# UT-Austin-RPL/GIGA

Hardware: AMD Instinct MI355X
Metric: scenes/sec (higher is better)
Workload: dtype f32; 1 GPU; c2: batch=32/GPU synthetic 40^3 TSDF, encoder + 3 grasp heads @1 query + occupancy head @2048 queries/scene (literal train_giga call), fp32 MFMA; parallelism=scene-sharded x1 (scene i -> rank i mod 1; replicas, no data-path collective)

## Files before the change

### giga_amd/csrc/giga_wino.h

```cpp
#pragma once
#include "giga_conv16.h"

namespace giga {

constexpr unsigned WINO_DEFAULT_MASK = 0xFFF;
constexpr int WINO_NW = 8;
constexpr int WINO_PS = 80;
template <int H, int W> struct WinoBlock {
    static constexpr int TW = W / 2, TH = H / 2;
    static constexpr int BW = TW % 4 == 0 ? 4 : 5, BH = TW % 4 == 0 ? 4 : 3;
    static constexpr int TXB = (TW + BW - 1) / BW, TYB = (TH + BH - 1) / BH;
    static constexpr int PW = 2 * BW + 2, PH = 2 * BH + 2;
    static constexpr int RS = BW == 4 ? 832 : 1040;
    static constexpr int REGION = PH * RS;
    static_assert(BW * BH <= 16 && PW * WINO_PS <= RS, "tile block");
};
constexpr int wino_kpass(int cin) { return cin > 64 ? cin / 64 : 1; }
template <int C0, int C1, int H, int W>
constexpr int wino_nw() {
    constexpr int CINP = (C0 + C1) / wino_kpass(C0 + C1);
    constexpr int fit = (160 * 1024 - 16 * CINP * 16 * 4) / WinoBlock<H, W>::REGION;
    return fit >= WINO_NW ? WINO_NW : (fit / 2) * 2;
}
template <int C0, int C1, int H, int W>
constexpr size_t wino_lds_bytes() {
    constexpr int CINP = (C0 + C1) / wino_kpass(C0 + C1);
    return (size_t)16 * CINP * 16 * 4 + (size_t)wino_nw<C0, C1, H, W>() * WinoBlock<H, W>::REGION;
}
constexpr size_t wino_image_bytes(int cin, int cout) { return (size_t)16 * cin * cout * 4; }

__device__ __forceinline__ void store_f32x4(float* uniform_base, unsigned byte_off, f32x4v v) {
    *reinterpret_cast<f32x4v*>(reinterpret_cast<char*>(uniform_base) + byte_off) = v;
}

template <int C0, int C1, int COUT>
__device__ __forceinline__ void wino_fill(const ConvArgs& a, uint8_t* smem, int block, int nblocks, int kpass) {
    constexpr int CIN = C0 + C1, KP = wino_kpass(CIN), CINP = CIN / KP, NGRP = COUT / 16;
    constexpr int WFRAGS = 16 * (CINP / 16);
    const int lane = threadIdx.x & 63;
    const int wave = __builtin_amdgcn_readfirstlane(threadIdx.x >> 6);
    const int nwl = blockDim.x >> 6;
    const int grp = conv_wg_map<NGRP>(a, block, nblocks).grp;
    const uint8_t* wsrc = a.w + ((size_t)grp * KP + kpass) * WFRAGS * FRAG;
    for (int c = wave; c < WFRAGS; c += nwl)
        __builtin_amdgcn_global_load_lds(
            (const __attribute__((address_space(1))) void*)(wsrc + (size_t)c * FRAG + lane * 16),
            (__attribute__((address_space(3))) void*)(smem + c * FRAG), 16, 0, 0);
}

template <int C0, int C1, int COUT, int H, int W, bool POOL, bool RELU>
__device__ __forceinline__ void wino_run(const ConvArgs& a, uint8_t* smem, int block, int nblocks, int kpass) {
    using G = WinoBlock<H, W>;
    constexpr int CIN = C0 + C1, KP = wino_kpass(CIN), CINP = CIN / KP, NCHUNK = CINP / 16, NGRP = COUT / 16;
    constexpr int NWV = wino_nw<C0, C1, H, W>();
    constexpr int BW = G::BW, BH = G::BH, PW = G::PW, PH = G::PH, RS = G::RS, PS = WINO_PS, REGION = G::REGION;
    constexpr int NVEC = PW * PH * 4, NLD = (NVEC + 63) / 64;
    constexpr int WBYTES = 16 * CINP * 16 * 4;
    static_assert(C1 == 0 || (C0 % 16 == 0 && (KP == 1 || C0 % CINP == 0)), "concat boundary on a chunk / pass boundary");
    static_assert(!POOL || KP == 1, "pooled layers are single-pass");
    static_assert(KP <= 2, "a third pass would read partials back through an L1 line it has read before");

    const int lane = threadIdx.x & 63;
    const int wave = __builtin_amdgcn_readfirstlane(threadIdx.x >> 6);
    const int j = lane & 15, g = lane >> 4;
    const bool active = wave < NWV;
    CONV_T(0);
    uint8_t* region = smem + WBYTES + (active ? wave : 0) * REGION;
    const ConvWgMap wm = conv_wg_map<NGRP>(a, block, nblocks);
    const int grp = wm.grp, wg_in_grp = wm.wg_in_grp, wgs_per_grp = wm.wgs_per_grp;
    const int units_all = wm.nimg * G::TYB * G::TXB;
    const int ulo = (int)((long long)units_all * wg_in_grp / wgs_per_grp), uhi = (int)((long long)units_all * (wg_in_grp + 1) / wgs_per_grp);
    const int units = uhi;
    const bool klast = kpass == KP - 1;

    const int jt = j < BW * BH ? j : 0;
    const int tyl = jt / BW, txl = jt % BW;
    const int a_off = 2 * tyl * RS + 2 * txl * PS + 16 * g;

    const int v16 = (lane & 3) * 16;
    const uint32_t rowb = (uint32_t)(a.cs0 ? a.cs0 : C0) * 4;
    constexpr uint32_t OOB = 0x80000000u;
    int st_lds[NLD];
    uint32_t st_rel[NLD];
#pragma unroll
    for (int q = 0; q < NLD; ++q) {
        const int i = lane + 64 * q, pix = i >> 2, ly = pix / PW, lx = pix % PW;
        st_lds[q] = i < NVEC ? ly * RS + lx * PS + v16 : 64;
        st_rel[q] = i < NVEC ? (uint32_t)(ly * W + lx) * rowb + (uint32_t)v16 : OOB;
    }
    const uint32_t in_bytes = (uint32_t)a.nimg * H * W * rowb;
    const __amdgpu_buffer_rsrc_t rs0 = __builtin_amdgcn_make_buffer_rsrc(
        const_cast<char*>(reinterpret_cast<const char*>(a.in0)) + (size_t)a.co0 * 4, 0, in_bytes, 0x00020000);
    const __amdgpu_buffer_rsrc_t rs1 = C1 > 0 ? __builtin_amdgcn_make_buffer_rsrc(
        const_cast<char*>(reinterpret_cast<const char*>(a.in1)) + (size_t)a.co1 * 4, 0, in_bytes, 0x00020000) : rs0;
    auto unit_coords = [&](int u, int& bx, int& by, int& img) {
        bx = u % G::TXB; by = (u / G::TXB) % G::TYB; img = wm.img0 + u / (G::TXB * G::TYB);
    };
    typedef unsigned u32x4v __attribute__((ext_vector_type(4)));
    u32x4v stg[NLD];
    uint32_t st_off[NLD];
    auto unit_setup = [&](int u) {
        int bx, by, img;
        unit_coords(u, bx, by, img);
        const int y0 = 2 * BH * by - 1, x0 = 2 * BW * bx - 1;
        const uint32_t base = (uint32_t)((img * H + y0) * W + x0) * rowb;
        if (y0 >= 0 && x0 >= 0 && y0 + PH <= H && x0 + PW <= W) {
#pragma unroll
            for (int q = 0; q < NLD; ++q) st_off[q] = (64 * (q + 1) > NVEC && st_rel[q] == OOB) ? OOB : st_rel[q] + base;
        } else {
#pragma unroll
            for (int q = 0; q < NLD; ++q) {
                const int pix = (lane >> 2) + 16 * q;
                const int ly = (pix * (65536 / PW + 1)) >> 16, lx = pix - ly * PW;
                const bool ok = st_rel[q] != OOB && (unsigned)(y0 + ly) < (unsigned)H && (unsigned)(x0 + lx) < (unsigned)W;
                st_off[q] = ok ? st_rel[q] + base : OOB;
            }
        }
    };
    auto issue_loads = [&](int cc) {
        const int c16 = kpass * CINP + cc * 16;
        const bool first = C1 == 0 || c16 < C0;
        const int soff = (first ? c16 : c16 - C0) * 4;
#pragma unroll
        for (int q = 0; q < NLD; ++q)
            stg[q] = first ? __builtin_amdgcn_raw_buffer_load_b128(rs0, st_off[q], soff, 0)
                           : __builtin_amdgcn_raw_buffer_load_b128(rs1, st_off[q], soff, 0);
    };

    int u = ulo + wave;
    const bool work = active && u < units;
    if (work) { unit_setup(u); issue_loads(0); }
    const f32x4v bias4 = (a.bias && klast) ? *reinterpret_cast<const f32x4v*>(a.bias + grp * 16 + 4 * g) : f32x4v{0.f, 0.f, 0.f, 0.f};
    __builtin_amdgcn_s_waitcnt(0x0F70);
    __syncthreads();
    if (!work) return;
    CONV_T(1);
    int tcount = 2;

    f32x4v acc[16];
    const uint8_t* wl = smem + lane * 8;
    float* outp = reinterpret_cast<float*>(a.out);

    auto epilogue = [&](const int u) {
        int bx, by, img;
        unit_coords(u, bx, by, img);
        const int ty = BH * by + tyl, tx = BW * bx + txl;
        const bool ok = j < BW * BH && ty < G::TH && tx < G::TW;
        f32x4v t0[4], t1[4];
#pragma unroll
        for (int xi = 0; xi < 4; ++xi) {
            t0[xi] = (acc[4 * xi] + acc[4 * xi + 1]) + acc[4 * xi + 2];
            t1[xi] = acc[4 * xi + 1] - (acc[4 * xi + 2] + acc[4 * xi + 3]);
        }
        f32x4v y[4];
        y[0] = (t0[0] + t0[1]) + t0[2]; y[1] = (t1[0] + t1[1]) + t1[2];
        y[2] = t0[1] - (t0[2] + t0[3]); y[3] = t1[1] - (t1[2] + t1[3]);
        const uint32_t pix = (uint32_t)((img * H + 2 * ty) * W + 2 * tx);
        const uint32_t o00 = (pix * COUT + grp * 16 + 4 * g) * 4u;
        if (ok) {
#pragma unroll
            for (int e = 0; e < 4; ++e) {
                const uint32_t off = o00 + (uint32_t)(((e >> 1) * W + (e & 1)) * COUT * 4);
                if constexpr (KP > 1) {
                    if (kpass > 0) y[e] += *reinterpret_cast<const f32x4v*>(reinterpret_cast<const char*>(outp) + off);
                }
                if (klast) {
                    if (RELU) {
#pragma unroll
                        for (int r = 0; r < 4; ++r) y[e][r] = relu(y[e][r]);
                    } else if (a.mask) {
                        const f32x4v mk = *reinterpret_cast<const f32x4v*>(reinterpret_cast<const char*>(a.mask) + off);
#pragma unroll
                        for (int r = 0; r < 4; ++r) y[e][r] = mk[r] > 0.f ? y[e][r] : 0.f;
                    }
                }
                store_f32x4(outp, off, y[e]);
            }
            if constexpr (POOL) {
                f32x4v mx;
#pragma unroll
                for (int r = 0; r < 4; ++r) mx[r] = fmaxf(fmaxf(y[0][r], y[1][r]), fmaxf(y[2][r], y[3][r]));
                const uint32_t pp = (uint32_t)((img * (H / 2) + ty) * (W / 2) + tx);
                store_f32x4(reinterpret_cast<float*>(a.out_pool), (pp * COUT + grp * 16 + 4 * g) * 4u, mx);
            }
        }
    };

    f32x2v d[4][4];
    auto load_d = [&](const int h) {
#pragma unroll
        for (int r = 0; r < 4; ++r)
#pragma unroll
            for (int x = 0; x < 4; ++x)
                d[r][x] = *(const volatile __attribute__((address_space(3))) f32x2v*)(region + a_off + r * RS + x * PS + 8 * h);
    };
    auto stage_write = [&]() {
#pragma unroll
        for (int q = 0; q < NLD; ++q) *reinterpret_cast<u32x4v*>(region + st_lds[q]) = stg[q];
    };
    f32x2v v[16];
    auto transform = [&]() {
#pragma unroll
        for (int x = 0; x < 4; ++x) {
            const f32x2v e0 = d[0][x] - d[2][x], e1 = d[1][x] + d[2][x], e2 = d[2][x] - d[1][x], e3 = d[1][x] - d[3][x];
            d[0][x] = e0; d[1][x] = e1; d[2][x] = e2; d[3][x] = e3;
        }
#pragma unroll
        for (int xi = 0; xi < 4; ++xi) {
            v[4 * xi + 0] = d[xi][0] - d[xi][2];
            v[4 * xi + 1] = d[xi][1] + d[xi][2];
            v[4 * xi + 2] = d[xi][2] - d[xi][1];
            v[4 * xi + 3] = d[xi][1] - d[xi][3];
        }
    };
    auto burst = [&](auto first_tag, const int cc, const int h, auto&& mid) {
        constexpr bool FIRST = decltype(first_tag)::value;
        const uint8_t* wbase = wl + (cc * 2 + h) * 512;
        constexpr int PD = 4;
        f32x2v wq[PD][2];
#pragma unroll
        for (int pp = 0; pp < PD; ++pp) {
            wq[pp][0] = *reinterpret_cast<const f32x2v*>(wbase + (2 * pp) * NCHUNK * 1024);
            wq[pp][1] = *reinterpret_cast<const f32x2v*>(wbase + (2 * pp + 1) * NCHUNK * 1024);
        }
        __builtin_amdgcn_sched_barrier(0);
#pragma unroll
        for (int pp = 0; pp < 8; ++pp) {
            const int sl = pp % PD, p0 = 2 * pp, p1 = 2 * pp + 1;
            if constexpr (FIRST) {
                acc[p0] = mfma32_16(wq[sl][0][0], v[p0][0], f32x4v{0.f, 0.f, 0.f, 0.f});
                acc[p1] = mfma32_16(wq[sl][1][0], v[p1][0], p1 == 5 ? bias4 : f32x4v{0.f, 0.f, 0.f, 0.f});
            } else {
                acc[p0] = mfma32_16(wq[sl][0][0], v[p0][0], acc[p0]);
                acc[p1] = mfma32_16(wq[sl][1][0], v[p1][0], acc[p1]);
            }
            acc[p0] = mfma32_16(wq[sl][0][1], v[p0][1], acc[p0]);
            acc[p1] = mfma32_16(wq[sl][1][1], v[p1][1], acc[p1]);
            __builtin_amdgcn_sched_barrier(0);
            if (pp + PD < 8) {
                wq[sl][0] = *reinterpret_cast<const f32x2v*>(wbase + (2 * (pp + PD)) * NCHUNK * 1024);
                wq[sl][1] = *reinterpret_cast<const f32x2v*>(wbase + (2 * (pp + PD) + 1) * NCHUNK * 1024);
            }
            if (pp == 3) mid();
            __builtin_amdgcn_sched_barrier(0);
        }
    };

    static_assert(NCHUNK >= 2, "loads run two chunks ahead");
    stage_write();
    issue_loads(1);
    load_d(0);
    while (true) {
        const int un = u + NWV;
        const bool more = un < units;
#pragma unroll
        for (int cc = 0; cc < NCHUNK; ++cc) {
            transform();
            auto mid0 = [&]() { load_d(1); };
            if (cc == 0) burst(std::true_type{}, cc, 0, mid0); else burst(std::false_type{}, cc, 0, mid0);
            if (cc == 0) { CONV_T(tcount); ++tcount; }
            transform();
            auto mid1 = [&]() {
                if (cc + 1 < NCHUNK) {
                    stage_write();
                    if (cc + 2 < NCHUNK) issue_loads(cc + 2);
                    else if (more) { unit_setup(un); issue_loads(0); }
                    load_d(0);
                } else if (more) {
                    stage_write();
                    issue_loads(1);
                    load_d(0);
                }
            };
            burst(std::false_type{}, cc, 1, mid1);
        }
        epilogue(u);
        CONV_T(tcount); ++tcount;
        if (!more) break;
        u = un;
    }
    CONV_T(63);
}

template <int C0, int C1, int COUT, int H, int W, bool POOL, bool RELU>
__global__ __launch_bounds__((wino_nw<C0, C1, H, W>() * 64)) void wino_kernel(ConvArgs a) {
    extern __shared__ __attribute__((aligned(16))) uint8_t smem[];
    constexpr int KP = wino_kpass(C0 + C1);
#pragma unroll
    for (int k = 0; k < KP; ++k) {
        if (k > 0) {
            __builtin_amdgcn_s_waitcnt(0x0F70);
            __syncthreads();
        }
        wino_fill<C0, C1, COUT>(a, smem, (int)blockIdx.x, (int)gridDim.x, k);
        wino_run<C0, C1, COUT, H, W, POOL, RELU>(a, smem, (int)blockIdx.x, (int)gridDim.x, k);
    }
}

template <int CIN, int COUT>
__device__ __forceinline__ void up_fill(const ConvArgs& a, uint8_t* smem, int block, int nblocks) {
    constexpr int KG = CIN / 16, NBT = COUT / 16;
    const int lane = threadIdx.x & 63;
    const int wave = __builtin_amdgcn_readfirstlane(threadIdx.x >> 6);
    const int nwl = blockDim.x >> 6;
    const int grp = conv_wg_map<NBT>(a, block, nblocks).grp;
    for (int c = wave; c < 4 * KG; c += nwl) {
        const int sub = c / KG, kg = c - sub * KG;
        __builtin_amdgcn_global_load_lds(
            (const __attribute__((address_space(1))) void*)(a.w + ((size_t)(sub * NBT + grp) * KG + kg) * FRAG + lane * 16),
            (__attribute__((address_space(3))) void*)(smem + c * FRAG), 16, 0, 0);
    }
}
template <int CIN, int COUT, int H, int W>
__device__ __forceinline__ void up_run(const ConvArgs& a, uint8_t* smem, int block, int nblocks) {
    constexpr int KG = CIN / 16, NBT = COUT / 16, NWV = WINO_NW;
    const int lane = threadIdx.x & 63;
    const int wave = __builtin_amdgcn_readfirstlane(threadIdx.x >> 6);
    const int j = lane & 15, g = lane >> 4;
    const bool active = wave < NWV;
    const ConvWgMap wm = conv_wg_map<NBT>(a, block, nblocks);
    const int grp = wm.grp;
    const int npix = wm.nimg * H * W, p0 = wm.img0 * H * W;
    const int units_all = (npix + 15) / 16;
    const int ulo = (int)((long long)units_all * wm.wg_in_grp / wm.wgs_per_grp), uhi = (int)((long long)units_all * (wm.wg_in_grp + 1) / wm.wgs_per_grp);
    const uint32_t rowb = (uint32_t)(a.cs0 ? a.cs0 : CIN) * 4;
    const char* in = reinterpret_cast<const char*>(a.in0) + (size_t)a.co0 * 4 + 16 * g;
    f32x4v x[2][KG];
    auto issue = [&](int u, f32x4v (&dst)[KG]) {
        int p = 16 * u + j;
        p = p < npix ? p : npix - 1;
        const char* q = in + (size_t)(p0 + p) * rowb;
#pragma unroll
        for (int k = 0; k < KG; ++k) dst[k] = *reinterpret_cast<const f32x4v*>(q + 64 * k);
    };
    int u = ulo + wave;
    const bool work = active && u < uhi;
    if (work) issue(u, x[0]);
    const f32x4v bias4 = a.bias ? *reinterpret_cast<const f32x4v*>(a.bias + grp * 16 + 4 * g) : f32x4v{0.f, 0.f, 0.f, 0.f};
    __builtin_amdgcn_s_waitcnt(0x0F70);
    __syncthreads();
    if (!work) return;
    const f32x4v* wl = reinterpret_cast<const f32x4v*>(smem) + lane;
    float* outp = reinterpret_cast<float*>(a.out);
    auto unit = [&](const int u, const f32x4v (&xb)[KG]) {
        f32x4v acc[4];
#pragma unroll
        for (int k = 0; k < KG; ++k) {
            f32x4v wv[4];
#pragma unroll
            for (int sub = 0; sub < 4; ++sub) wv[sub] = wl[(sub * KG + k) * 64];
#pragma unroll
            for (int e = 0; e < 4; ++e)
#pragma unroll
                for (int sub = 0; sub < 4; ++sub)
                    acc[sub] = (k == 0 && e == 0) ? mfma32_16(wv[sub][e], xb[k][e], bias4) : mfma32_16(wv[sub][e], xb[k][e], acc[sub]);
        }
        const int p = 16 * u + j;
        if (p < npix) {
            const int pg = p0 + p, img = pg / (H * W), r = pg - img * (H * W), y = r / W, xx = r - y * W;
            const uint32_t o00 = ((uint32_t)((img * 2 * H + 2 * y) * 2 * W + 2 * xx) * COUT + grp * 16 + 4 * g) * 4u;
#pragma unroll
            for (int sub = 0; sub < 4; ++sub)
                store_f32x4(outp, o00 + (uint32_t)(((sub >> 1) * 2 * W + (sub & 1)) * COUT * 4), acc[sub]);
        }
    };
    while (true) {
        const int un = u + NWV;
        const bool more = un < uhi;
        if (more) issue(un, x[1]);
        unit(u, x[0]);
        if (!more) break;
        const int un2 = un + NWV;
        const bool more2 = un2 < uhi;
        if (more2) issue(un2, x[0]);
        unit(un, x[1]);
        if (!more2) break;
        u = un2;
    }
}
template <int CIN, int COUT>
constexpr size_t up_lds_bytes() { return (size_t)4 * (CIN / 16) * FRAG; }
template <int CIN, int COUT, int H, int W>
__global__ __launch_bounds__(WINO_NW * 64) void up_kernel(ConvArgs a) {
    extern __shared__ __attribute__((aligned(16))) uint8_t smem[];
    up_fill<CIN, COUT>(a, smem, (int)blockIdx.x, (int)gridDim.x);
    up_run<CIN, COUT, H, W>(a, smem, (int)blockIdx.x, (int)gridDim.x);
}
template <int CIN, int COUT, int H, int W>
inline int launch_up(const ConvArgs& a, hipStream_t s) {
    constexpr int NBT = COUT / 16;
    constexpr size_t lds = up_lds_bytes<CIN, COUT>();
    const size_t in_pix = (size_t)a.nimg * H * W;
    if (in_pix * 4 >= (1u << 24) || in_pix * 4 * COUT * 4 >= (1ull << 32)) return -7;
    const int units = (int)((in_pix + 15) / 16);
    int wgs = (units + WINO_NW - 1) / WINO_NW;
    if (wgs > 256 / NBT) wgs = 256 / NBT;
    else if (a.xcd_local && a.nimg % 8 == 0 && wgs % 8 != 0 && wgs + 8 - wgs % 8 <= 256 / NBT) wgs += 8 - wgs % 8;
    auto kern = up_kernel<CIN, COUT, H, W>;
    if (lds > 48 * 1024) giga::dyn_lds_once(reinterpret_cast<const void*>(kern), (int)lds);
    GIGA_LAUNCH(kern, dim3(wgs * NBT), dim3(WINO_NW * 64), lds, s, a);
    return hipGetLastError() == hipSuccess ? 0 : -10;
}

template <int C0, int C1, int COUT, int H, int W, bool POOL, bool RELU = true>
inline int launch_wino(const ConvArgs& a, hipStream_t s) {
    using G = WinoBlock<H, W>;
    constexpr int NWV = wino_nw<C0, C1, H, W>(), NGRP = COUT / 16;
    constexpr size_t lds = wino_lds_bytes<C0, C1, H, W>();
    static_assert(lds <= 160 * 1024 && NWV >= 4, "LDS budget");
    static_assert(256 % NGRP == 0, "weight groups must divide the CU count");
    const size_t in_pix = (size_t)a.nimg * H * W;
    if (C1 > 0 && (a.cs0 ? a.cs0 : C0) != (a.cs1 ? a.cs1 : C1)) return -7;
    if (in_pix * (size_t)((a.cs0 ? a.cs0 : C0) * 4) >= (1ull << 31)) return -7;
    if (in_pix >= (1u << 24) || in_pix * (size_t)((a.cs0 ? a.cs0 : C0) * 4) >= (1ull << 32) ||
        (C1 > 0 && in_pix * (size_t)((a.cs1 ? a.cs1 : C1) * 4) >= (1ull << 32)) || in_pix * COUT * 4 >= (1ull << 32)) return -7;
    const int units = a.nimg * G::TXB * G::TYB;
    int wgs = (units + NWV - 1) / NWV;
    if (wgs > 256 / NGRP) wgs = 256 / NGRP;
    else if (a.xcd_local && a.nimg % 8 == 0 && wgs % 8 != 0 && wgs + 8 - wgs % 8 <= 256 / NGRP) wgs += 8 - wgs % 8;
    auto kern = wino_kernel<C0, C1, COUT, H, W, POOL, RELU>;
    if (lds > 48 * 1024) giga::dyn_lds_once(reinterpret_cast<const void*>(kern), (int)lds);
    GIGA_LAUNCH(kern, dim3(wgs * NGRP), dim3(NWV * 64), lds, s, a);
    return hipGetLastError() == hipSuccess ? 0 : -10;
}

}
```

Before: 98200 scenes/s.

## Precompute per-boundary-class halo load offsets in an LDS table for Winograd conv

Per-unit computation of halo-load offsets and bounds checks is replaced by a small LDS table, one entry per boundary class (first, interior, last block in x and y). Each unit now adds a per-unit scalar base and reads its offsets from the table ahead of time. The buffer resource base is shifted back by one row plus one pixel so the offsets stay non-negative. The output transform is split into paired 2-wide ops with asm barriers to steer codegen, and the `more` test is recomputed through an opaque asm. The table costs extra LDS, which may lower the wave count in LDS-bound configurations.

```diff
diff --git a/giga_amd/csrc/giga_wino.h b/giga_amd/csrc/giga_wino.h
--- a/giga_amd/csrc/giga_wino.h
+++ b/giga_amd/csrc/giga_wino.h
@@ -14,21 +14,29 @@
     static constexpr int RS = BW == 4 ? 832 : 1040;
     static constexpr int REGION = PH * RS;
     static_assert(BW * BH <= 16 && PW * WINO_PS <= RS, "tile block");
+    static constexpr int NCX = TXB < 3 ? TXB : 3, NCY = TYB < 3 ? TYB : 3, NCLS = NCX * NCY;
+    static constexpr int NLD = (PW * PH * 4 + 63) / 64;
+    static constexpr int TAB = NCLS * NLD * 256;
+    static constexpr int cls(int b, int nb, int nc) { return b == 0 ? 0 : b == nb - 1 ? nc - 1 : 1; }
+    static constexpr int rep(int c, int nb, int nc) { return c == 0 ? 0 : c == nc - 1 ? nb - 1 : 1; }
+    static_assert((TXB < 3 || (2 * BW - 1 >= 0 && 2 * BW * (TXB - 2) - 1 + PW <= W)) &&
+                  (TYB < 3 || (2 * BH - 1 >= 0 && 2 * BH * (TYB - 2) - 1 + PH <= H)), "blocks between the first and the last lie inside the image");
 };
 constexpr int wino_kpass(int cin) { return cin > 64 ? cin / 64 : 1; }
 template <int C0, int C1, int H, int W>
 constexpr int wino_nw() {
     constexpr int CINP = (C0 + C1) / wino_kpass(C0 + C1);
-    constexpr int fit = (160 * 1024 - 16 * CINP * 16 * 4) / WinoBlock<H, W>::REGION;
+    constexpr int fit = (160 * 1024 - 16 * CINP * 16 * 4 - WinoBlock<H, W>::TAB) / WinoBlock<H, W>::REGION;
     return fit >= WINO_NW ? WINO_NW : (fit / 2) * 2;
 }
 template <int C0, int C1, int H, int W>
 constexpr size_t wino_lds_bytes() {
     constexpr int CINP = (C0 + C1) / wino_kpass(C0 + C1);
-    return (size_t)16 * CINP * 16 * 4 + (size_t)wino_nw<C0, C1, H, W>() * WinoBlock<H, W>::REGION;
+    return (size_t)16 * CINP * 16 * 4 + (size_t)wino_nw<C0, C1, H, W>() * WinoBlock<H, W>::REGION + WinoBlock<H, W>::TAB;
 }
 constexpr size_t wino_image_bytes(int cin, int cout) { return (size_t)16 * cin * cout * 4; }
 
+__device__ __forceinline__ f32x2v pair_of(f32x4v a, int hh) { return hh ? f32x2v{a[2], a[3]} : f32x2v{a[0], a[1]}; }
 __device__ __forceinline__ void store_f32x4(float* uniform_base, unsigned byte_off, f32x4v v) {
     *reinterpret_cast<f32x4v*>(reinterpret_cast<char*>(uniform_base) + byte_off) = v;
 }
@@ -54,7 +62,7 @@
     constexpr int CIN = C0 + C1, KP = wino_kpass(CIN), CINP = CIN / KP, NCHUNK = CINP / 16, NGRP = COUT / 16;
     constexpr int NWV = wino_nw<C0, C1, H, W>();
     constexpr int BW = G::BW, BH = G::BH, PW = G::PW, PH = G::PH, RS = G::RS, PS = WINO_PS, REGION = G::REGION;
-    constexpr int NVEC = PW * PH * 4, NLD = (NVEC + 63) / 64;
+    constexpr int NVEC = PW * PH * 4, NLD = G::NLD;
     constexpr int WBYTES = 16 * CINP * 16 * 4;
     static_assert(C1 == 0 || (C0 % 16 == 0 && (KP == 1 || C0 % CINP == 0)), "concat boundary on a chunk / pass boundary");
     static_assert(!POOL || KP == 1, "pooled layers are single-pass");
@@ -81,55 +89,83 @@
     const uint32_t rowb = (uint32_t)(a.cs0 ? a.cs0 : C0) * 4;
     constexpr uint32_t OOB = 0x80000000u;
     int st_lds[NLD];
-    uint32_t st_rel[NLD];
 #pragma unroll
     for (int q = 0; q < NLD; ++q) {
         const int i = lane + 64 * q, pix = i >> 2, ly = pix / PW, lx = pix % PW;
         st_lds[q] = i < NVEC ? ly * RS + lx * PS + v16 : 64;
-        st_rel[q] = i < NVEC ? (uint32_t)(ly * W + lx) * rowb + (uint32_t)v16 : OOB;
-    }
-    const uint32_t in_bytes = (uint32_t)a.nimg * H * W * rowb;
+    }
+    auto st_entry = [&](int q, int x0, int y0) -> uint32_t {
+        const int i = lane + 64 * q, pix = i >> 2;
+        const int ly = (pix * (65536 / PW + 1)) >> 16, lx = pix - ly * PW;
+        const bool ok = i < NVEC && (unsigned)(y0 + ly) < (unsigned)H && (unsigned)(x0 + lx) < (unsigned)W;
+        return ok ? (uint32_t)(ly * W + lx) * rowb + (uint32_t)v16 : OOB;
+    };
+    const uint32_t front = (uint32_t)(W + 1) * rowb;
+    const uint32_t in_bytes = (uint32_t)a.nimg * H * W * rowb + front;
     const __amdgpu_buffer_rsrc_t rs0 = __builtin_amdgcn_make_buffer_rsrc(
-        const_cast<char*>(reinterpret_cast<const char*>(a.in0)) + (size_t)a.co0 * 4, 0, in_bytes, 0x00020000);
+        const_cast<char*>(reinterpret_cast<const char*>(a.in0)) + (size_t)a.co0 * 4 - front, 0, in_bytes, 0x00020000);
     const __amdgpu_buffer_rsrc_t rs1 = C1 > 0 ? __builtin_amdgcn_make_buffer_rsrc(
-        const_cast<char*>(reinterpret_cast<const char*>(a.in1)) + (size_t)a.co1 * 4, 0, in_bytes, 0x00020000) : rs0;
+        const_cast<char*>(reinterpret_cast<const char*>(a.in1)) + (size_t)a.co1 * 4 - front, 0, in_bytes, 0x00020000) : rs0;
     auto unit_coords = [&](int u, int& bx, int& by, int& img) {
         bx = u % G::TXB; by = (u / G::TXB) % G::TYB; img = wm.img0 + u / (G::TXB * G::TYB);
+    };
+    auto unit_base = [&](int u) -> uint32_t {
+        int bx, by, img;
+        unit_coords(u, bx, by, img);
+        return (uint32_t)((img * H + 2 * BH * by) * W + 2 * BW * bx) * rowb;
+    };
+    constexpr int TAB0 = WBYTES + NWV * REGION;
+    typedef const __attribute__((address_space(3))) uint32_t* tab_ptr;
+    const tab_ptr tab_lane = (tab_ptr)(smem + TAB0 + lane * 4);
+    auto unit_tab = [&](int u) -> tab_ptr {
+        int bx, by, img;
+        unit_coords(u, bx, by, img);
+        return tab_lane + (G::cls(by, G::TYB, G::NCY) * G::NCX + G::cls(bx, G::TXB, G::NCX)) * (NLD * 64);
     };
     typedef unsigned u32x4v __attribute__((ext_vector_type(4)));
     u32x4v stg[NLD];
     uint32_t st_off[NLD];
-    auto unit_setup = [&](int u) {
-        int bx, by, img;
-        unit_coords(u, bx, by, img);
-        const int y0 = 2 * BH * by - 1, x0 = 2 * BW * bx - 1;
-        const uint32_t base = (uint32_t)((img * H + y0) * W + x0) * rowb;
-        if (y0 >= 0 && x0 >= 0 && y0 + PH <= H && x0 + PW <= W) {
-#pragma unroll
-            for (int q = 0; q < NLD; ++q) st_off[q] = (64 * (q + 1) > NVEC && st_rel[q] == OOB) ? OOB : st_rel[q] + base;
-        } else {
-#pragma unroll
-            for (int q = 0; q < NLD; ++q) {
-                const int pix = (lane >> 2) + 16 * q;
-                const int ly = (pix * (65536 / PW + 1)) >> 16, lx = pix - ly * PW;
-                const bool ok = st_rel[q] != OOB && (unsigned)(y0 + ly) < (unsigned)H && (unsigned)(x0 + lx) < (unsigned)W;
-                st_off[q] = ok ? st_rel[q] + base : OOB;
-            }
-        }
+    uint32_t sbase = 0;
+    tab_ptr tab_next = tab_lane;
+    auto unit_read = [&]() {
+#pragma unroll
+        for (int q = 0; q < NLD; ++q) st_off[q] = tab_next[q * 64];
     };
     auto issue_loads = [&](int cc) {
         const int c16 = kpass * CINP + cc * 16;
         const bool first = C1 == 0 || c16 < C0;
-        const int soff = (first ? c16 : c16 - C0) * 4;
+        const int coff = (first ? c16 : c16 - C0) * 4;
 #pragma unroll
         for (int q = 0; q < NLD; ++q)
-            stg[q] = first ? __builtin_amdgcn_raw_buffer_load_b128(rs0, st_off[q], soff, 0)
-                           : __builtin_amdgcn_raw_buffer_load_b128(rs1, st_off[q], soff, 0);
+            stg[q] = first ? __builtin_amdgcn_raw_buffer_load_b128(rs0, st_off[q] + coff, sbase, 0)
+                           : __builtin_amdgcn_raw_buffer_load_b128(rs1, st_off[q] + coff, sbase, 0);
     };
 
     int u = ulo + wave;
     const bool work = active && u < units;
-    if (work) { unit_setup(u); issue_loads(0); }
+    if (work) {
+        int bx, by, img;
+        unit_coords(u, bx, by, img);
+        sbase = unit_base(u);
+#pragma unroll
+        for (int q = 0; q < NLD; ++q) st_off[q] = st_entry(q, 2 * BW * bx - 1, 2 * BH * by - 1);
+        issue_loads(0);
+        tab_next = unit_tab(u + NWV);
+    }
+    for (int q = wave; q < NLD; q += (int)(blockDim.x >> 6)) {
+        const int i = lane + 64 * q, pix = i >> 2;
+        const int ly = (pix * (65536 / PW + 1)) >> 16, lx = pix - ly * PW;
+        const uint32_t rel = (uint32_t)(ly * W + lx) * rowb + (uint32_t)v16;
+#pragma unroll
+        for (int cy = 0; cy < G::NCY; ++cy) {
+            const bool oky = i < NVEC && (unsigned)(2 * BH * G::rep(cy, G::TYB, G::NCY) - 1 + ly) < (unsigned)H;
+#pragma unroll
+            for (int cx = 0; cx < G::NCX; ++cx) {
+                const bool okx = (unsigned)(2 * BW * G::rep(cx, G::TXB, G::NCX) - 1 + lx) < (unsigned)W;
+                *reinterpret_cast<uint32_t*>(smem + TAB0 + ((cy * G::NCX + cx) * NLD + q) * 256 + lane * 4) = oky && okx ? rel : OOB;
+            }
+        }
+    }
     const f32x4v bias4 = (a.bias && klast) ? *reinterpret_cast<const f32x4v*>(a.bias + grp * 16 + 4 * g) : f32x4v{0.f, 0.f, 0.f, 0.f};
     __builtin_amdgcn_s_waitcnt(0x0F70);
     __syncthreads();
@@ -146,15 +182,22 @@
         unit_coords(u, bx, by, img);
         const int ty = BH * by + tyl, tx = BW * bx + txl;
         const bool ok = j < BW * BH && ty < G::TH && tx < G::TW;
-        f32x4v t0[4], t1[4];
-#pragma unroll
-        for (int xi = 0; xi < 4; ++xi) {
-            t0[xi] = (acc[4 * xi] + acc[4 * xi + 1]) + acc[4 * xi + 2];
-            t1[xi] = acc[4 * xi + 1] - (acc[4 * xi + 2] + acc[4 * xi + 3]);
-        }
+        auto sub2 = [](f32x2v a, f32x2v b) { asm("" : "+v"(b)); f32x2v r = a - b; asm("" : "+v"(r)); return r; };
         f32x4v y[4];
-        y[0] = (t0[0] + t0[1]) + t0[2]; y[1] = (t1[0] + t1[1]) + t1[2];
-        y[2] = t0[1] - (t0[2] + t0[3]); y[3] = t1[1] - (t1[2] + t1[3]);
+#pragma unroll
+        for (int hh = 0; hh < 2; ++hh) {
+            f32x2v t0[4], t1[4];
+#pragma unroll
+            for (int xi = 0; xi < 4; ++xi) {
+                const f32x2v a0 = pair_of(acc[4 * xi], hh), a1 = pair_of(acc[4 * xi + 1], hh), a2 = pair_of(acc[4 * xi + 2], hh), a3 = pair_of(acc[4 * xi + 3], hh);
+                t0[xi] = (a0 + a1) + a2;
+                t1[xi] = sub2(a1, a2 + a3);
+            }
+            const f32x2v y0 = (t0[0] + t0[1]) + t0[2], y1 = (t1[0] + t1[1]) + t1[2];
+            const f32x2v y2 = sub2(t0[1], t0[2] + t0[3]), y3 = sub2(t1[1], t1[2] + t1[3]);
+            y[0][2 * hh] = y0[0]; y[0][2 * hh + 1] = y0[1]; y[1][2 * hh] = y1[0]; y[1][2 * hh + 1] = y1[1];
+            y[2][2 * hh] = y2[0]; y[2][2 * hh + 1] = y2[1]; y[3][2 * hh] = y3[0]; y[3][2 * hh + 1] = y3[1];
+        }
         const uint32_t pix = (uint32_t)((img * H + 2 * ty) * W + 2 * tx);
         const uint32_t o00 = (pix * COUT + grp * 16 + 4 * g) * 4u;
         if (ok) {
@@ -199,7 +242,7 @@
         for (int q = 0; q < NLD; ++q) *reinterpret_cast<u32x4v*>(region + st_lds[q]) = stg[q];
     };
     f32x2v v[16];
-    auto transform = [&]() {
+    auto transform = [&](auto after_burst_tag) {
 #pragma unroll
         for (int x = 0; x < 4; ++x) {
             const f32x2v e0 = d[0][x] - d[2][x], e1 = d[1][x] + d[2][x], e2 = d[2][x] - d[1][x], e3 = d[1][x] - d[3][x];
@@ -252,21 +295,24 @@
     load_d(0);
     while (true) {
         const int un = u + NWV;
-        const bool more = un < units;
+        auto more_now = [&]() { int t = un; asm volatile("" : "+s"(t)); return t < units; };
 #pragma unroll
         for (int cc = 0; cc < NCHUNK; ++cc) {
-            transform();
-            auto mid0 = [&]() { load_d(1); };
+            if (cc == 0) transform(std::false_type{}); else transform(std::true_type{});
+            auto mid0 = [&]() {
+                load_d(1);
+                if (cc + 2 == NCHUNK) { if (more_now()) unit_read(); }
+            };
             if (cc == 0) burst(std::true_type{}, cc, 0, mid0); else burst(std::false_type{}, cc, 0, mid0);
             if (cc == 0) { CONV_T(tcount); ++tcount; }
-            transform();
+            transform(std::true_type{});
             auto mid1 = [&]() {
                 if (cc + 1 < NCHUNK) {
                     stage_write();
                     if (cc + 2 < NCHUNK) issue_loads(cc + 2);
-                    else if (more) { unit_setup(un); issue_loads(0); }
+                    else if (more_now()) { sbase = unit_base(un); issue_loads(0); }
                     load_d(0);
-                } else if (more) {
+                } else if (more_now()) {
                     stage_write();
                     issue_loads(1);
                     load_d(0);
@@ -276,8 +322,10 @@
         }
         epilogue(u);
         CONV_T(tcount); ++tcount;
-        if (!more) break;
+        if (!more_now()) break;
         u = un;
+        tab_next = unit_tab(u + NWV);
+        asm volatile("" : "+v"(tab_next));
     }
     CONV_T(63);
 }
@@ -411,7 +459,7 @@
     static_assert(256 % NGRP == 0, "weight groups must divide the CU count");
     const size_t in_pix = (size_t)a.nimg * H * W;
     if (C1 > 0 && (a.cs0 ? a.cs0 : C0) != (a.cs1 ? a.cs1 : C1)) return -7;
-    if (in_pix * (size_t)((a.cs0 ? a.cs0 : C0) * 4) >= (1ull << 31)) return -7;
+    if ((in_pix + W + 1) * (size_t)((a.cs0 ? a.cs0 : C0) * 4) >= (1ull << 31)) return -7;
     if (in_pix >= (1u << 24) || in_pix * (size_t)((a.cs0 ? a.cs0 : C0) * 4) >= (1ull << 32) ||
         (C1 > 0 && in_pix * (size_t)((a.cs1 ? a.cs1 : C1) * 4) >= (1ull << 32)) || in_pix * COUT * 4 >= (1ull << 32)) return -7;
     const int units = a.nimg * G::TXB * G::TYB;
```

Measured after the change: 98920 scenes/s (median of 6 runs). No clear change (+0.7%).
